# probabilists/azula

Measured on AMD Instinct MI355X. Metric: images/sec (whole node), DDIM-64 256x256 UNet, higher is better.
Workload: dtype f32 (f16x2 split: 2 half pieces per operand, 3 partial products, f32 accumulate)

## Files before the change

### azula_amd/_lib.py

```python

from __future__ import annotations

import ctypes as C
import functools
import os
import threading

import torch

_HERE = os.path.dirname(os.path.abspath(__file__))
LIB_PATH = os.environ.get("AZULA_AMD_LIB") or os.path.join(_HERE, "csrc", "libazula_amd.so")

c_f32p = C.c_void_p
c_stream = C.c_void_p


class AzStepCoef(C.Structure):
    _fields_ = [
        ("c_in", C.c_float),
        ("c_skip", C.c_float),
        ("c_out", C.c_float),
        ("c_time", C.c_float),
        ("alpha_t", C.c_float),
        ("alpha_s", C.c_float),
# ... 408 lines not shown
    "az_adm_precond_bwd_in_f32": [vp, vp, vp, vp, vp, vp, i32, i64, i64, f32, f32, c_stream],
    "az_linear_small_f32": [vp, i64, vp, i64, vp, vp, i64, i64, i64, i32, i32, c_stream],
    "az_gather_rows_f32": [vp, vp, vp, i64, i64, i64, c_stream],
    "az_gather_step_row_f32": [vp, vp, vp, i32, i64, i64, c_stream],
    "az_coef_c_time_f32": [vp, vp, c_stream],
    "az_groupnorm_stats_f32": [vp, vp, vp, i64, i64, i64, i64, i64, i32, i32, c_stream],
    "az_groupnorm_finalize_f32": [C.POINTER(AzNormFinalizeArgs), c_stream],
    "az_affine_act_f32": [vp, vp, vp, i64, vp, vp, i64, i64, i64, i64, i32, i32, c_stream],
    "az_rownorm_mod_f32": [vp, vp, vp, vp, vp, i64, i64, i64, i64, i64, i32, f32, c_stream],
    "az_rownorm_mod_h16": [vp, vp, vp, vp, vp, i64, i64, i64, i64, i64, i32, f32, i32, c_stream],
    "az_groupnorm_stats_h16": [vp, vp, vp, i64, i64, i64, i64, i64, i32, i32, i32, c_stream],
    "az_affine_act_h16": [vp, vp, vp, i64, vp, vp, i64, i64, i64, i64, i32, i32, i32, c_stream],
    "az_token_copy_f32": [vp, i64, i64, vp, i64, i64, i64, i64, i64, c_stream],
    "az_token_fill_f32": [vp, i64, i64, i64, vp, i64, vp, i64, i64, c_stream],
    "az_token_fill_h16": [vp, i64, i64, i64, vp, i64, vp, i64, i64, i32, c_stream],
    "az_timestep_embedding_f32": [vp, i64, vp, i64, i64, i32, f32, c_stream],
    "az_linear_small_grouped_f32": [vp, i32, i32, i64, i32, i32, c_stream],
    "az_conv2d_f32": [C.POINTER(AzConvArgs), c_stream],
    "az_conv2d_stem_f32": [C.POINTER(AzConvArgs), c_stream],
    "az_conv2d_bf16_f32": [C.POINTER(AzConvArgs), c_stream],
    "az_conv2d_x3_f32": [C.POINTER(AzConvArgs), c_stream],
    "az_conv2d_f16_f32": [C.POINTER(AzConvArgs), c_stream],
    "az_pack_conv_weight_half_f32": [vp, vp, i32, i32, i32, i32, i32, i32, i32, i32, c_stream],
    "az_pack_conv_weight_x3_f32": [vp, vp, i32, i32, i32, i32, i32, i32, i32, c_stream],
    "az_conv2d_suggest_splitk": [i64, i32, i32, i32],
    "az_conv2d_x3_suggest_splitk": [C.POINTER(AzConvArgs)],
    "az_conv2d_winograd_f32": [C.POINTER(AzConvArgs), c_stream],
    "az_conv2d_winograd_suggest_splitk": [i64, i32, i32, i32, i32],
    "az_winograd_pack_filter_f32": [vp, vp, i32, i32, i32, i32, i32, i32, c_stream],
    "az_conv2d_winograd_x3_f32": [C.POINTER(AzConvArgs), c_stream],
    "az_winograd_pack_filter_x3_f32": [vp, vp, i32, i32, i32, i32, i32, i32, c_stream],
    "az_winograd_x3_choose_block": [i32, i32, i32, i32, vp, vp, vp, vp],
    "az_winograd_x3_block_geometry": [i32, i32, i32, i32, i32, i32, i32, vp, vp],
    "az_conv2d_f16x2_f32": [C.POINTER(AzConvArgs), c_stream],
    "az_conv2d_winograd_f16x2_f32": [C.POINTER(AzConvArgs), c_stream],
    "az_pack_conv_weight_f16x2_f32": [vp, vp, i32, i32, i32, i32, i32, i32, i32, f32, c_stream],
    "az_winograd_pack_filter_f16x2_f32": [vp, vp, i32, i32, i32, i32, i32, i32, f32, c_stream],
    "az_f16x2_weight_scale": [f32, i32],
    "az_absmax_f32": [vp, vp, i64, c_stream],
    "az_absmax_from_moments_f32": [vp, vp, i64, c_stream],
    "az_conv2d_winograd4_f32": [C.POINTER(AzConvArgs), c_stream],
    "az_conv2d_winograd4_suggest_splitk": [i64, i32, i32, i32, i32],
    "az_winograd4_pack_filter_f32": [vp, vp, i32, i32, i32, i32, i32, i32, c_stream],
    "az_pack_conv_weight_f32": [vp, vp, i32, i32, i32, i32, i32, i32, i32, c_stream],
    "az_attention_f32": [C.POINTER(AzAttnArgs), c_stream],
    "az_attention_x3_f32": [C.POINTER(AzAttnArgs), c_stream],
    "az_attention_f16x2_f32": [C.POINTER(AzAttnArgs), c_stream],
    "az_attention_bf16_f32": [C.POINTER(AzAttnArgs), c_stream],
    "az_attention_f16_f32": [C.POINTER(AzAttnArgs), c_stream],
    "az_qk_prep_f32": [vp, vp, vp, vp, i64, i64, i32, i32, i64, i64, i64, i64, i64, i64, i32, i32, f32, vp, vp, c_stream],
    "az_qk_prep_w_f32": [vp, vp, vp, vp, i64, i64, i32, i32, i64, i64, i64, i64, i64, i64, i32, i32, f32, vp, vp, vp, vp, c_stream],
    "az_qk_prep_bwd_f32": [vp, vp, vp, vp, vp, vp, i64, i64, i32, i32, i64, i64, i64, i64, i64, i64, i64, i64, i64, i32, i32, f32, vp, vp,
                           c_stream],
    "az_qk_prep_bwd_w_f32": [vp, vp, vp, vp, vp, vp, i64, i64, i32, i32, i64, i64, i64, i64, i64, i64, i64, i64, i64, i32, i32, f32, vp,
                             vp, vp, vp, c_stream],
    "az_attention_bwd_f32": [C.POINTER(AzAttnBwdArgs), c_stream],
    "az_swiglu_f32": [vp, vp, i64, i64, i64, i64, c_stream],
    "az_patchify_f32": [vp, vp, vp, i64, i64, i64, i64, i64, i64, c_stream],
    "az_unpatchify_f32": [vp, vp, i64, i64, i64, i64, i64, i64, c_stream],
    "az_graph_begin": [c_stream],
    "az_graph_end": [c_stream, C.POINTER(vp)],
    "az_graph_launch": [vp, c_stream],
    "az_graph_destroy": [vp],
    "az_graph_num_nodes": [vp, C.POINTER(i64)],
    "az_transition_f64": [C.POINTER(AzTransitionArgs), c_stream],
    "az_step_row_f64": [vp, vp, vp, i32, i32, c_stream],
# ... 75 lines not shown
```

### azula_amd/csrc/conv.hip

```cpp
#include "conv_shared.h"
#include <cstdio>
#include <cstdlib>
#include <type_traits>

namespace {

constexpr int BM = 128;
constexpr int BN = 128;
constexpr int BK = 32;
constexpr int LDSS = 36;
constexpr int TILE_F = (BM + BN) * LDSS;

#include "igemm_kloop.inc"
struct ConvP {
  AzConvArgs a;
  int npix;
  int cin_s;
  int nkc0;
  int nkc1;
  int nk;
  int kps;
  int tiles_m;
  int tiles_n;
  int asm_loop;
// ... 2625 lines not shown

int az_winograd_x3_choose_block(int32_t batch, int32_t hin, int32_t win, int32_t whole, int32_t* rect_w, int32_t* rect_h,
                                int64_t* slots, int64_t* slots_run) {
  AZ_REQUIRE(rect_w && rect_h && slots && slots_run, AZ_E_NULL);
  AZ_REQUIRE(batch > 0 && hin > 0 && win > 0 && (int64_t)batch * hin * win < (1ll << 31), AZ_E_SHAPE);
  int rw, rh;
  int64_t run;
  *slots = x3_choose_block(batch, (hin + 1) / 2, (win + 1) / 2, whole != 0, rw, rh, run);
  *rect_w = rw, *rect_h = rh, *slots_run = run;
  return AZ_OK;
}

int az_winograd_x3_block_geometry(int32_t batch, int32_t hin, int32_t win, int32_t pad_mode, int32_t rect_w, int32_t rect_h,
                                  int32_t block, int32_t* slot_pix, int32_t* tile_info) {
  AZ_REQUIRE(slot_pix && tile_info, AZ_E_NULL);
  AZ_REQUIRE(batch > 0 && hin > 0 && win > 0 && (int64_t)batch * hin * win < (1ll << 31), AZ_E_SHAPE);
  AZ_REQUIRE(rect_h > 1 && x3_shape_ok(rect_w, rect_h), AZ_E_UNSUPPORTED);
  const int tiles_h = (hin + 1) / 2, tiles_w = (win + 1) / 2;
  AZ_REQUIRE(block >= 0 && block < (int64_t)batch * x3_rect_blocks_per_image(tiles_h, tiles_w, rect_w, rect_h), AZ_E_SHAPE);
  const X3RectGeom g = x3_rect_geom(block, tiles_h, tiles_w, rect_w, rect_h);
  for (int s = 0; s < 512; ++s) {
    int ih, iw;
    const bool ok = x3_rect_slot_pixel(g, s, hin, win, pad_mode, ih, iw);
    slot_pix[3 * s] = ok ? g.b : -1, slot_pix[3 * s + 1] = ok ? ih : -1, slot_pix[3 * s + 2] = ok ? iw : -1;
  }
  for (int j = 0; j < WT; ++j) {
    int th, tw, ps;
    const bool ok = x3_rect_tile(g, j, tiles_h, tiles_w, th, tw, ps);
    tile_info[4 * j] = ok ? g.b : -1, tile_info[4 * j + 1] = th, tile_info[4 * j + 2] = tw, tile_info[4 * j + 3] = ps;
  }
  return g.nslots;
}

static int winograd_x3_entry(const AzConvArgs* a, az_stream_t stream, bool h2) {
  WinoP p;
  int splitk = 1;
  const int prc = wino_prepare(a, 16, 16ll * WC * 16 * 3 * 2, p, splitk);
  if (prc != AZ_OK) return prc;
  AZ_REQUIRE(p.tiles_w >= 2, AZ_E_UNSUPPORTED);
  {
    const bool whole = p.a.gn_quads != nullptr;
    int rw, rh;
    int64_t run_slots;
    x3_choose_block(a->batch, p.tiles_h, p.tiles_w, whole, rw, rh, run_slots);
    if (const char* e = az_ab_env("AZ_X3_BLOCK")) {
      int ew = 0, eh = 0;
      if (sscanf(e, "%d,%d", &ew, &eh) == 2) {
        AZ_REQUIRE(x3_shape_ok(ew, eh) && !(whole && eh > 1 && (p.tiles_w % ew || p.tiles_h % eh)), AZ_E_UNSUPPORTED);
        rw = ew, rh = eh;
      }
    }
    if (rh > 1) {
      p.rect_w = rw, p.rect_h = rh;
      p.tblocks = a->batch * x3_rect_blocks_per_image(p.tiles_h, p.tiles_w, rw, rh);
      wino_order(p, 16);
    }
  }
  if (h2) AZ_REQUIRE(conv_pow2(a->w_scale), AZ_E_SHAPE);
  p.out_scale = h2 ? 1.f / a->w_scale : 1.f;
  if (h2) AZ_REQUIRE(AZ_ALIGNED16(a->in_absmax0) && AZ_ALIGNED16(a->in_absmax1) && (a->in_absmax0 || !a->in_absmax1), AZ_E_ALIGN);
  hipStream_t st = az_s(stream);
  int rc = azi_winograd_x3_launch(p, (unsigned)splitk, st, h2);
  if (rc != AZ_OK) return rc;
  if (splitk > 1) {
    ConvP cp;
    cp.a = p.a;
    cp.a.gn_quads = a->gn_quads;
    cp.npix = p.npix;
    rc = launch_splitk_reduce(cp, st);
  }
  return rc;
}

static void wino_order(WinoP& p, int wk) {
  int env_gt = 0, env_gc = 0;
  if (const char* e = az_ab_env("AZ_WINO_RECT")) sscanf(e, "%d,%d", &env_gt, &env_gc);
  int gt = env_gt > 0 ? env_gt : 8, gc = env_gt > 0 ? (env_gc > 0 ? env_gc : p.cblocks) : (wk == 16 ? 2 : 4);
  while (gc > 1 && p.cblocks % gc) gc >>= 1;
  if (env_gt <= 0) gt = 32 / gc;
  while (gt > 1 && p.tblocks % gt) gt >>= 1;
  if (p.cblocks % gc || p.tblocks % gt) gt = 1, gc = p.cblocks;
  p.gt = gt, p.gc = gc;
}

static int wino_prepare(const AzConvArgs* a, int wk, int64_t ustage_bytes, WinoP& p, int& splitk) {
  AZ_REQUIRE(a && a->src0 && a->weight && a->dst, AZ_E_NULL);
  AZ_REQUIRE(a->ksize == 3 && a->stride == 1 && a->pad == 1 && !a->aniso && a->src_dtype == 0 && a->dst_dtype == 0, AZ_E_UNSUPPORTED);
  AZ_REQUIRE(a->batch > 0 && a->hin > 0 && a->win > 0 && a->hout == a->hin && a->wout == a->win, AZ_E_SHAPE);
  AZ_REQUIRE(a->c0s > 0 && a->c0s % 4 == 0 && a->c1s % 4 == 0 && a->cout_s > 0 && a->cout_s % 4 == 0, AZ_E_SHAPE);
  AZ_REQUIRE((a->c1s == 0) == (a->src1 == nullptr), AZ_E_SHAPE);
// ... 31 lines not shown
  const int64_t npix64 = (int64_t)a->batch * a->hout * a->wout;
  AZ_REQUIRE(npix64 < (1ll << 31), AZ_E_SHAPE);
  if (a->gn_quads && a->splitk == 1) {
    const int64_t tiles_img = (int64_t)((a->hout + 1) / 2) * ((a->wout + 1) / 2);
    AZ_REQUIRE(!a->dst_nchw && a->cout_s % WC == 0 && tiles_img % WT == 0 && a->hout % 2 == 0 &&
                   a->wout % 2 == 0 && a->gn_chunks == tiles_img / WT,
               AZ_E_UNSUPPORTED);
  }

  p.a = *a;
  p.npix = (int)npix64;
  p.tiles_h = (a->hout + 1) / 2;
  p.tiles_w = (a->wout + 1) / 2;
  p.ntiles = a->batch * p.tiles_h * p.tiles_w;
  p.nkc0 = (a->c0s + wk - 1) / wk;
  p.nkc1 = (a->c1s + wk - 1) / wk;
  p.nk = p.nkc0 + p.nkc1;
  {
    const int64_t tiles_img = (int64_t)p.tiles_h * p.tiles_w;
    const int64_t span = (WT + tiles_img - 1) / tiles_img + 1;
    AZ_REQUIRE(span * a->h0 * a->w0 * a->c0s * 4 < (1ll << 31), AZ_E_SHAPE);
    AZ_REQUIRE(span * a->h1 * a->w1 * a->c1s * 4 < (1ll << 31), AZ_E_SHAPE);
  }
  splitk = a->splitk;
  if (splitk > p.nk) splitk = p.nk;
  p.kps = (p.nk + splitk - 1) / splitk;
  splitk = (p.nk + p.kps - 1) / p.kps;
  p.a.splitk = splitk;
  AZ_REQUIRE(!a->gn_quads || (a->splitk == 1) == (splitk == 1), AZ_E_UNSUPPORTED);
  if (splitk > 1) p.a.gn_quads = nullptr;
  p.cblocks = (a->cout_s + WC - 1) / WC;
  p.tblocks = (p.ntiles + WT - 1) / WT;
  p.rect_w = WT, p.rect_h = 1;
  wino_order(p, wk);
  AZ_REQUIRE((int64_t)p.nk * p.cblocks * ustage_bytes <= (1ll << 31), AZ_E_SHAPE);
  return AZ_OK;
}

int az_conv2d_winograd_suggest_splitk(int64_t batch, int32_t hout, int32_t wout, int32_t cout_s, int32_t cin_s) {
  const int64_t tiles = batch * ((hout + 1) / 2) * ((wout + 1) / 2);
  const int64_t blocks = ((tiles + WT - 1) / WT) * ((cout_s + WC - 1) / WC);
  const int64_t nk = (cin_s + WK - 1) / WK;
  int64_t want = (256 + blocks - 1) / blocks;
  int64_t maxs = nk / 8;
  if (maxs < 1) maxs = 1;
  if (want > maxs) want = maxs;
  if (want > 16) want = 16;
  if (blocks >= 192) want = 1;
  return (int)(want < 1 ? 1 : want);
}

int az_conv2d_winograd4_f32(const AzConvArgs* a, az_stream_t stream) {
  AZ_REQUIRE(a && a->src0 && a->weight && a->dst, AZ_E_NULL);
  AZ_REQUIRE(a->ksize == 3 && a->stride == 1 && a->pad == 1 && !a->aniso && a->src_dtype == 0 && a->dst_dtype == 0, AZ_E_UNSUPPORTED);
  AZ_REQUIRE(a->batch > 0 && a->hin > 0 && a->win > 0 && a->hout == a->hin && a->wout == a->win, AZ_E_SHAPE);
  AZ_REQUIRE(a->c0s > 0 && a->c0s % 4 == 0 && a->c1s % 4 == 0 && a->cout_s > 0 && a->cout_s % 4 == 0, AZ_E_SHAPE);
  AZ_REQUIRE((a->c1s == 0) == (a->src1 == nullptr), AZ_E_SHAPE);
  AZ_REQUIRE((a->act >= 0 && a->act <= 4) || a->act == 6, AZ_E_UNSUPPORTED);
  if (a->act == 6) AZ_REQUIRE(a->res && !a->gate && !a->dst_nchw && !a->gn_quads, AZ_E_UNSUPPORTED);
  if (a->act == 4) AZ_REQUIRE(!a->gate && !a->res && !a->dst_nchw && !a->gn_quads && a->cout_s % 8 == 0, AZ_E_UNSUPPORTED);
  AZ_REQUIRE(!a->in_affine && a->depth == 0, AZ_E_UNSUPPORTED);
  AZ_REQUIRE(!a->aniso || (a->up0_w >= 0 && a->up0_w <= 4 && a->up1_w >= 0 && a->up1_w <= 4), AZ_E_SHAPE);
  AZ_REQUIRE(a->up0 >= 0 && a->up0 <= 4 && ((a->hin + (1 << a->up0) - 1) >> a->up0) <= a->h0 &&
                 ((a->win + (1 << az_upw(a, a->up0, a->up0_w)) - 1) >> az_upw(a, a->up0, a->up0_w)) <= a->w0,
             AZ_E_SHAPE);
  if (a->src1)
// ... 73 lines not shown
```

### azula_amd/csrc/conv_shared.h

```cpp
#pragma once

#include "common.h"

namespace {

typedef float f32x16 __attribute__((ext_vector_type(16)));

__device__ __forceinline__ float4 ld4(const float* p) { return *reinterpret_cast<const float4*>(p); }


typedef unsigned int u32x4 __attribute__((ext_vector_type(4)));

__device__ __forceinline__ float4 buf_ld4(__amdgpu_buffer_rsrc_t rsrc, unsigned voff, unsigned soff) {
  const u32x4 v = __builtin_amdgcn_raw_buffer_load_b128(rsrc, (int)voff, (int)soff, 0);
  return __builtin_bit_cast(float4, v);
}

typedef float f32x2 __attribute__((ext_vector_type(2)));
typedef unsigned int u32x2 __attribute__((ext_vector_type(2)));

__device__ __forceinline__ f32x2 buf_ld2(__amdgpu_buffer_rsrc_t rsrc, unsigned voff, unsigned soff) {
  const u32x2 v = __builtin_amdgcn_raw_buffer_load_b64(rsrc, (int)voff, (int)soff, 0);
  return __builtin_bit_cast(f32x2, v);
}
// ... 323 lines not shown
  return az_fdiv(tiles_h + rh - 1, rh) * az_fdiv(tiles_w + rw - 1, rw);
}

__host__ __device__ __forceinline__ X3RectGeom x3_rect_geom(int tb, int tiles_h, int tiles_w, int rw, int rh) {
  X3RectGeom g;
  g.rw = rw, g.rh = rh;
  g.ws = 2 * rw + 2;
  g.nslots = (2 * rh + 2) * g.ws;
  const int bw = az_fdiv(tiles_w + rw - 1, rw);
  const int bpi = az_fdiv(tiles_h + rh - 1, rh) * bw;
  g.b = az_fdiv(tb, bpi);
  g.rb = tb - g.b * bpi;
  const int by = az_fdiv(g.rb, bw);
  g.th0 = by * rh;
  g.tw0 = (g.rb - by * bw) * rw;
  return g;
}

__host__ __device__ __forceinline__ bool x3_rect_slot_pixel(const X3RectGeom& g, int s, int hin, int win, int pad_mode, int& ih, int& iw) {
  const int r = az_fdiv(s, g.ws);
  ih = wrap_coord(2 * g.th0 - 1 + r, hin, pad_mode);
  iw = wrap_coord(2 * g.tw0 - 1 + (s - r * g.ws), win, pad_mode);
  return s < g.nslots && (unsigned)ih < (unsigned)hin && (unsigned)iw < (unsigned)win;
}

__host__ __device__ __forceinline__ bool x3_rect_tile(const X3RectGeom& g, int j, int tiles_h, int tiles_w, int& th, int& tw, int& pslot) {
  const int jy = az_fdiv(j, g.rw), jx = j - jy * g.rw;
  th = g.th0 + jy;
  tw = g.tw0 + jx;
  pslot = 2 * jy * g.ws + 2 * jx;
  return th < tiles_h && tw < tiles_w;
}


}

struct WinoP {
  AzConvArgs a;
  int npix;
  int tiles_h, tiles_w, ntiles;
  int nkc0, nkc1, nk;
  int kps;
  int cblocks;
  int tblocks;
  int gt, gc;
  int rect_w, rect_h;
  float out_scale;
};
```

### azula_amd/csrc/wino_x3.hip

```cpp
#include "conv_shared.h"

#include <cstdlib>
#include <type_traits>

namespace {

typedef __bf16 bf16x8 __attribute__((ext_vector_type(8)));
typedef _Float16 f16x8 __attribute__((ext_vector_type(8)));

constexpr int XT = 64;
constexpr int XC = 64;
constexpr int XK = 16;
constexpr int X_ROW = XK * 4;
constexpr int X_FREQ = XT * X_ROW;
constexpr int X_HALF = 8 * X_FREQ;
constexpr int X_STAGE = 2 * X_HALF;
constexpr int X_SLOTS = 768;
constexpr int X_SLOT = 64;
constexpr int X_DOFF1 = X_STAGE + X_SLOTS * X_SLOT;
constexpr int X_OT = 2 * XC + 4;
constexpr int X_EPI_BYTES = (4 * XT * X_OT + 3 * XT + 384) * 4;
constexpr int X_LDS_BYTES = X_DOFF1 + 512 * 32 > X_EPI_BYTES ? X_DOFF1 + 512 * 32 : X_EPI_BYTES;
static_assert(X_LDS_BYTES >= X_DOFF1 + 512 * 32 && X_LDS_BYTES >= 4 * 128 * 64 * 4, "the epilogue reuses the K loop's LDS");
constexpr int XU_STEP_BYTES = 16 * XC * XK * 3 * 2;
static_assert(4 * X_SLOTS <= 6 * 512, "six staging pieces per thread");
static_assert(X_LDS_BYTES <= 160 * 1024, "one workgroup per CU");

template <int AFF, bool TAIL, bool H2 = false, bool RECT = false>
__global__ __launch_bounds__(512, 2) void conv_winograd_x3_kernel(WinoP p) {
  extern __shared__ __attribute__((aligned(16))) float wsm[];
  char* const smem = reinterpret_cast<char*>(wsm);
  const AzConvArgs& a = p.a;
  const int tid = threadIdx.x;
  const int lane = tid & 63;
  const int wave = tid >> 6;
  const int wxi = wave & 3;
  const int wk = wave >> 2;
  const int l31 = lane & 31;
  const int h = lane >> 5;

  const int nwg = gridDim.x;
  const int bid = blockIdx.x;
  const int xq = nwg >> 3, xr = nwg & 7, xcd = bid & 7;
  const int wg = (xcd < xr ? xcd * (xq + 1) : xr * (xq + 1) + (xcd - xr) * xq) + (bid >> 3);
  const int rsz = p.gt * p.gc;
  const int rect = wg / rsz, rin = wg - rect * rsz;
  const int rcols = p.cblocks / p.gc;
  const int rrow = rect / rcols;
  const int rin_c = rin / p.gt;
  const int tb = rrow * p.gt + (rin - rin_c * p.gt);
  const int cb = (rect - rrow * rcols) * p.gc + rin_c;
  const int t0 = tb * XT;
  const int tiles_img = p.tiles_h * p.tiles_w;
  X3RectGeom rg = {};
  if constexpr (RECT) rg = x3_rect_geom(tb, p.tiles_h, p.tiles_w, p.rect_w, p.rect_h);
  const int b_first = RECT ? rg.b : t0 / tiles_img;

  const int kt_begin = blockIdx.y * p.kps;
  const int kt_end = min(p.nk, kt_begin + p.kps);
  const float pin = H2 ? az_f16x2_in_scale(a.in_absmax0, a.in_absmax1, 4.f, lane) : 1.f;
  const float pin2k = pin * 2048.f;
// ... 136 lines not shown
#pragma unroll
      for (int c = 0; c < 4; ++c) rv[4 * r + c] = *reinterpret_cast<const f32x2*>(patch + r * prow + c * X_SLOT);
  };
  const __amdgpu_buffer_rsrc_t raf = __builtin_amdgcn_make_buffer_rsrc(
      (void*)(AFF != 0 ? a.in_affine : nullptr), 0, AFF != 0 ? (unsigned)(2 * a.batch * a.c0s * 4) : 0u, 0x00020000);
  const unsigned af_voff = (unsigned)(((b_first + (v_b < 0 ? 0 : v_b)) * a.c0s + vq * 2) * 4);
  const unsigned af_shift = (unsigned)(a.batch * a.c0s * 4);
  f32x2 af_sc = {0.f, 0.f}, af_sh = {0.f, 0.f};
  auto affine_load = [&](int kt) __attribute__((always_inline)) {
    if constexpr (AFF != 0) {
      const bool kv = !TAIL || kt * XK + vq * 2 < a.c0s;
      af_sc = buf_ld2(raf, kv ? af_voff : OOB, (unsigned)(kt * XK * 4));
      af_sh = buf_ld2(raf, kv ? af_voff : OOB, (unsigned)(kt * XK * 4) + af_shift);
    }
  };
  auto affine = [&]() __attribute__((always_inline)) {
    if constexpr (AFF != 0) {
#pragma unroll
      for (int i = 0; i < 16; ++i) {
        f32x2 v = rv[i] * af_sc + af_sh;
        if constexpr (AFF == 2) v = f32x2{az_silu(v.x), az_silu(v.y)};
        rv[i] = (vmask >> i) & 1u ? v : f32x2{0.f, 0.f};
      }
    }
  };
  auto row_transform = [&](int c) __attribute__((always_inline)) {
    const f32x2 d0 = rv[c], d1 = rv[4 + c], d2 = rv[8 + c], d3 = rv[12 + c];
    rv[c] = d0 - d2;
    rv[4 + c] = d1 + d2;
    rv[8 + c] = d2 - d1;
    rv[12 + c] = d1 - d3;
  };
  const int vrow = vj * X_ROW + (((vq >> 1) ^ ((vj >> 2) & 3)) * 16) + (vq & 1) * 8;
  auto nu_store = [&](int hs, int xi) __attribute__((always_inline)) {
    const f32x2 u0 = rv[4 * xi], u1 = rv[4 * xi + 1], u2 = rv[4 * xi + 2], u3 = rv[4 * xi + 3];
    char* dst = smem + hs * X_HALF + vrow + (2 * xi) * X_FREQ;
    *reinterpret_cast<f32x2*>(dst) = hs == 0 ? u0 - u2 : u2 - u1;
    *reinterpret_cast<f32x2*>(dst + X_FREQ) = hs == 0 ? u1 + u2 : u1 - u3;
  };
  const unsigned u_lane = (unsigned)(lane * 16);
  constexpr bool H2_DERIVE = true;
  uint4 ua[2][3];
  typedef _Float16 f16x8v __attribute__((ext_vector_type(8)));
  auto derive_u2 = [&]() __attribute__((always_inline)) {
#pragma unroll
    for (int ch = 0; ch < 2; ++ch) ua[ch][2] = __builtin_bit_cast(uint4, __builtin_bit_cast(f16x8v, ua[ch][0]) * (_Float16)0.00048828125f);
  };
  auto load_u = [&](int kt, int f, int pl) __attribute__((always_inline)) {
    const unsigned soff =
        (unsigned)__builtin_amdgcn_readfirstlane((int)((((int64_t)kt * p.cblocks + cb) * 8 + wave) * (12 * 1024) + f * (6 * 1024)));
#pragma unroll
    for (int ch = 0; ch < 2; ++ch) ua[ch][pl] = __builtin_bit_cast(uint4, buf_ld4(rw, u_lane + (unsigned)((ch * 3 + pl) * 1024), soff));
  };

  f32x16 acc[8];
#pragma unroll
  for (int f = 0; f < 8; ++f)
#pragma unroll
    for (int r = 0; r < 16; ++r) acc[f][r] = 0.f;

  const int fragB = (2 * wxi + wk) * X_FREQ + l31 * X_ROW;
  const int fsw = (l31 >> 2) & 3;
  float xf[2][8];
  unsigned fw[2][3][4];
  auto frag_read = [&](int hs, int th) __attribute__((always_inline)) {
    const char* vb = smem + hs * X_HALF + fragB + th * (32 * X_ROW);
    const float4 lo = *reinterpret_cast<const float4*>(vb + (((2 * h) ^ fsw) * 16));
    const float4 hi = *reinterpret_cast<const float4*>(vb + (((2 * h + 1) ^ fsw) * 16));
    xf[th][0] = lo.x, xf[th][1] = lo.y, xf[th][2] = lo.z, xf[th][3] = lo.w;
// ... 11 lines not shown
      xf[th][i] = x - __builtin_bit_cast(float, __builtin_bit_cast(unsigned, x) & 0xFFFF0000u);
    }
  };
  constexpr int PA[6] = {H2 ? 1 : 2, H2 ? 0 : 1, H2 ? 2 : 0, 1, 0, 0};
  constexpr int PB[6] = {0, 0, H2 ? 1 : 0, 1, 1, 2};
  auto mf = [&](int f, int k) __attribute__((always_inline)) {
    const int t = k >> 2, th = (k >> 1) & 1, ch = k & 1;
    f32x16& c = acc[4 * f + 2 * ch + th];
    uint4 bw = make_uint4(fw[th][PB[t]][0], fw[th][PB[t]][1], fw[th][PB[t]][2], fw[th][PB[t]][3]);
    if constexpr (H2) c = __builtin_amdgcn_mfma_f32_32x32x16_f16(__builtin_bit_cast(f16x8, ua[ch][PA[t]]), __builtin_bit_cast(f16x8, bw), c, 0, 0, 0);
    else c = __builtin_amdgcn_mfma_f32_32x32x16_bf16(__builtin_bit_cast(bf16x8, ua[ch][PA[t]]), __builtin_bit_cast(bf16x8, bw), c, 0, 0, 0);
  };
  typedef _Float16 h2v __attribute__((ext_vector_type(2)));
  auto h_piece = [&](int th) __attribute__((always_inline)) {
#pragma unroll
    for (int j = 0; j < 4; ++j) {
      const f32x2 x = {xf[th][2 * j], xf[th][2 * j + 1]};
      const f32x2 v = x * pin;
      fw[th][0][j] = __builtin_bit_cast(unsigned, __builtin_convertvector(v, h2v));
      const f32x2 t = x * pin2k;
      xf[th][2 * j] = t.x, xf[th][2 * j + 1] = t.y;
    }
  };
  auto l_piece = [&](int th) __attribute__((always_inline)) {
#pragma unroll
    for (int j = 0; j < 4; ++j) {
      const h2v hh = __builtin_bit_cast(h2v, fw[th][0][j]);
      const h2v l = {(_Float16)__builtin_fmaf((float)hh.x, -2048.f, xf[th][2 * j]), (_Float16)__builtin_fmaf((float)hh.y, -2048.f, xf[th][2 * j + 1])};
      fw[th][1][j] = __builtin_bit_cast(unsigned, l);
    }
  };

#define XS_FENCE __builtin_amdgcn_sched_barrier(0)
  auto phase = [&](auto HS, int kt, int ktn) __attribute__((always_inline)) {
    constexpr int hs = decltype(HS)::value;
    constexpr int ob = 1 - hs;
    const int ktu = hs == 0 ? kt : ktn;
    if constexpr (H2) {
      h_piece(0); XS_FENCE;
      if constexpr (hs == 0) {
        mf(hs, 0); h_piece(1); XS_FENCE;
        mf(hs, 1); nu_store(ob, 0); nu_store(ob, 1); XS_FENCE;
        mf(hs, 2); nu_store(ob, 2); nu_store(ob, 3); gl(ktn, 0); gl(ktn, 1); gl(ktn, 2); XS_FENCE;
        mf(hs, 3); gl(ktn, 3); gl(ktn, 4); gl(ktn, 5); load_u(ktu, ob, 1); XS_FENCE;
        mf(hs, 4); l_piece(0); XS_FENCE;
        mf(hs, 5); l_piece(1); if constexpr (H2_DERIVE) derive_u2(); XS_FENCE;
        mf(hs, 6); XS_FENCE;
        mf(hs, 7); load_u(ktu, ob, 0); XS_FENCE;
        mf(hs, 8); gs(0); XS_FENCE;
        mf(hs, 9); gs(1); gs(2); XS_FENCE;
        mf(hs, 10); gs(3); gs(4); XS_FENCE;
        mf(hs, 11); gs(5);
      } else {
        mf(hs, 0); h_piece(1); affine_load(ktn); XS_FENCE;
        mf(hs, 1); patch_rows(ktn, 0, 2); XS_FENCE;
        mf(hs, 2); patch_rows(ktn, 2, 4); XS_FENCE;
        mf(hs, 3); l_piece(0); load_u(ktu, ob, 1); XS_FENCE;
        mf(hs, 4); l_piece(1); if constexpr (H2_DERIVE) derive_u2(); XS_FENCE;
        affine();
        mf(hs, 5); row_transform(0); row_transform(1); XS_FENCE;
        mf(hs, 6); row_transform(2); row_transform(3); XS_FENCE;
        mf(hs, 7); load_u(ktu, ob, 0); XS_FENCE;
        mf(hs, 8); nu_store(ob, 0); XS_FENCE;
        mf(hs, 9); nu_store(ob, 1); XS_FENCE;
        mf(hs, 10); nu_store(ob, 2); XS_FENCE;
        mf(hs, 11); nu_store(ob, 3);
      }
      if constexpr (!H2_DERIVE) load_u(ktu, ob, 2);
// ... 27 lines not shown
    } else {
      mf(hs, 0); piece(1, 0); XS_FENCE;
      mf(hs, 1); affine_load(ktn); remainder(0, 0, 2); XS_FENCE;
      mf(hs, 2); remainder(0, 2, 4); XS_FENCE;
      mf(hs, 3); remainder(1, 0, 2); XS_FENCE;
      mf(hs, 4); remainder(1, 2, 4); load_u(ktu, ob, 2); XS_FENCE;
      mf(hs, 5); piece(0, 1); XS_FENCE;
      mf(hs, 6); piece(1, 1); XS_FENCE;
      mf(hs, 7); remainder(0, 0, 2); XS_FENCE;
      mf(hs, 8); remainder(0, 2, 4); XS_FENCE;
      mf(hs, 9); remainder(1, 0, 2); XS_FENCE;
      mf(hs, 10); remainder(1, 2, 4); XS_FENCE;
      mf(hs, 11); piece(0, 2); piece(1, 2); XS_FENCE;
      mf(hs, 12); patch_rows(ktn, 0, 2); XS_FENCE;
      mf(hs, 13); patch_rows(ktn, 2, 4); XS_FENCE;
      mf(hs, 14); XS_FENCE;
      mf(hs, 15); XS_FENCE;
      mf(hs, 16); load_u(ktu, ob, 1); XS_FENCE;
      affine();
      mf(hs, 17); row_transform(0); row_transform(1); XS_FENCE;
      mf(hs, 18); row_transform(2); row_transform(3); XS_FENCE;
      mf(hs, 19); nu_store(ob, 0); XS_FENCE;
      mf(hs, 20); nu_store(ob, 1); XS_FENCE;
      mf(hs, 21); nu_store(ob, 2); XS_FENCE;
      mf(hs, 22); nu_store(ob, 3); XS_FENCE;
      mf(hs, 23);
    }
    load_u(ktu, ob, 0);
    }
    __syncthreads();
    frag_read(ob, 0); frag_read(ob, 1);
    XS_FENCE;
  };

  if (kt_begin < kt_end) {
#pragma unroll
    for (int m = 0; m < 6; ++m) gl(kt_begin, m);
    if constexpr (H2) {
      XS_FENCE; load_u(kt_begin, 0, 1); XS_FENCE; load_u(kt_begin, 0, 0); XS_FENCE;
      if constexpr (!H2_DERIVE) { load_u(kt_begin, 0, 2); XS_FENCE; }
    } else {
      XS_FENCE; load_u(kt_begin, 0, 2); XS_FENCE; load_u(kt_begin, 0, 1); XS_FENCE; load_u(kt_begin, 0, 0); XS_FENCE;
    }
#pragma unroll
    for (int m = 0; m < 6; ++m) gs(m);
    __syncthreads();
    affine_load(kt_begin);
    patch_rows(kt_begin, 0, 4);
    affine();
#pragma unroll
    for (int c = 0; c < 4; ++c) row_transform(c);
#pragma unroll
    for (int xi = 0; xi < 4; ++xi) nu_store(0, xi);
    __syncthreads();
    frag_read(0, 0); frag_read(0, 1);
    if (wave >= 4) __builtin_amdgcn_s_setprio(1);
#pragma unroll 1
    for (int kt = kt_begin; kt < kt_end; ++kt) {
      const int ktn = min(kt + 1, kt_end - 1);
      if (ktn >= p.nkc0 && cur_src == 0) switch_source();
      phase(std::integral_constant<int, 0>{}, kt, ktn);
      phase(std::integral_constant<int, 1>{}, kt, ktn);
    }
    __builtin_amdgcn_s_setprio(0);
  }
  __syncthreads();
#undef XS_FENCE
  if constexpr (H2) {
    const float osc = __fdiv_rn(p.out_scale, pin);
#pragma unroll
    for (int q = 0; q < 8; ++q) acc[q] = acc[q] * osc;
  }

  if (wk == 0) {
    asm volatile("" ::: "memory");
#pragma unroll
    for (int q = 0; q < 4; ++q) {
      acc[q] = acc[q] + acc[4 + q];
      acc[4 + q] = -acc[4 + q];
    }
  } else {
    asm volatile("" ::: "memory");
#pragma unroll
    for (int q = 0; q < 4; ++q) acc[4 + q] = acc[q] - acc[4 + q];
  }
  {
    float4* hand = reinterpret_cast<float4*>(wsm) + wxi * (32 * 64) + lane;
    if (wk == 1) {
#pragma unroll
      for (int q = 0; q < 8; ++q)
#pragma unroll
        for (int g = 0; g < 4; ++g) hand[(q * 4 + g) * 64] = make_float4(acc[q][4 * g], acc[q][4 * g + 1], acc[q][4 * g + 2], acc[q][4 * g + 3]);
    }
    __syncthreads();
    if (wk == 0) {
// ... 84 lines not shown
    a2 = (a2 + b2) + d * d * half_n;
  };
  chan(am, a2, __shfl_xor(am, 16), __shfl_xor(a2, 16), 16.f);
  chan(am, a2, __shfl_xor(am, 32), __shfl_xor(a2, 32), 32.f);
  float* sh = reinterpret_cast<float*>(tinfo + 3 * XT);
  if (lane < 16) {
    sh[wave * 16 + lane] = am;
    sh[128 + wave * 16 + lane] = a2;
  }
  __syncthreads();
  if (tid < 16) {
    float wm[8], w2[8];
#pragma unroll
    for (int k = 0; k < 8; ++k) {
      wm[k] = sh[k * 16 + tid];
      w2[k] = sh[128 + k * 16 + tid];
    }
    float hn = 64.f;
#pragma unroll
    for (int o = 1; o < 8; o <<= 1, hn *= 2.f)
#pragma unroll
      for (int k = 0; k < 8; k += 2 * o) chan(wm[k], w2[k], wm[k + o], w2[k + o], hn);
    const int chunk = RECT ? rg.rb : (t0 - b_first * tiles_img) / XT;
    float* out = a.gn_quads + ((((int64_t)b_first * a.gn_chunks + chunk) * (a.cout_s / 4)) + (cb * (XC / 4) + tid)) * 4;
    out[0] = 1024.f;
    out[1] = wm[0];
    out[2] = w2[0];
    out[3] = 0.f;
  }
}

}

template <int AFF, bool TAIL, bool H2, bool RECT>
static int launch_x3(const WinoP& p, unsigned splitk, hipStream_t st) {
  static std::atomic<uint64_t> lds_set{0};
  hipError_t e = az_max_dynamic_lds((const void*)conv_winograd_x3_kernel<AFF, TAIL, H2, RECT>, X_LDS_BYTES, lds_set);
  if (e != hipSuccess) return (int)e;
  hipLaunchKernelGGL((conv_winograd_x3_kernel<AFF, TAIL, H2, RECT>), dim3((unsigned)((int64_t)p.cblocks * p.tblocks), splitk), dim3(512), X_LDS_BYTES,
                     st, p);
  return az_launch_status();
}

template <bool H2, bool RECT>
static int launch_x3_mode(const WinoP& p, unsigned splitk, hipStream_t st) {
  const bool tail = (p.a.c0s % XK) != 0 || (p.a.c1s % XK) != 0;
  const int aff = !p.a.in_affine ? 0 : (p.a.in_act == 0 ? 1 : 2);
  switch (aff * 2 + (tail ? 1 : 0)) {
    case 0: return launch_x3<0, false, H2, RECT>(p, splitk, st);
    case 1: return launch_x3<0, true, H2, RECT>(p, splitk, st);
    case 2: return launch_x3<1, false, H2, RECT>(p, splitk, st);
    case 3: return launch_x3<1, true, H2, RECT>(p, splitk, st);
    case 4: return launch_x3<2, false, H2, RECT>(p, splitk, st);
    default: return launch_x3<2, true, H2, RECT>(p, splitk, st);
  }
}

__attribute__((visibility("hidden"))) int azi_winograd_x3_launch(const WinoP& p, unsigned splitk, hipStream_t st, bool h2) {
  if (p.rect_h > 1) {
    if (p.rect_w * p.rect_h != XT || (2 * p.rect_w + 2) * (2 * p.rect_h + 2) > 512) return AZ_E_SHAPE;
    return h2 ? launch_x3_mode<true, true>(p, splitk, st) : launch_x3_mode<false, true>(p, splitk, st);
  }
  return h2 ? launch_x3_mode<true, false>(p, splitk, st) : launch_x3_mode<false, false>(p, splitk, st);
}
```

### include/azula_amd.h

```cpp
#ifndef AZULA_AMD_H
#define AZULA_AMD_H

#include <stdint.h>

#ifdef __cplusplus
extern "C" {
#endif

#define AZ_VERSION 1

enum {
  AZ_OK = 0,
  AZ_E_NULL = -1,
  AZ_E_SHAPE = -2,
  AZ_E_ALIGN = -3,
  AZ_E_UNSUPPORTED = -4
};

typedef void* az_stream_t;

int az_version(void);
const char* az_error_string(int code);

typedef struct AzStepCoef {
// ... 316 lines not shown
  int32_t src_dtype;
  int32_t depth;
  int32_t depth_shift;
  int32_t qk_head_dim;
  int32_t qk_heads;
  int32_t qk_tokens;
  int32_t qk_rmsnorm;
  float qk_eps;
  int32_t qk_reserved;
  const float* qk_q_weight;
  const float* qk_k_weight;
  const float* qk_rope_cos;
  const float* qk_rope_sin;
  int32_t depth_wrap;
  int32_t dst_dtype;
  float w_scale;
  int32_t reserved1;
  const float* in_absmax0;
  const float* in_absmax1;
} AzConvArgs;
int az_conv2d_f32(const AzConvArgs* args, az_stream_t stream);
int az_conv2d_stem_f32(const AzConvArgs* args, az_stream_t stream);
int az_conv2d_bf16_f32(const AzConvArgs* args, az_stream_t stream);
int az_conv2d_f16_f32(const AzConvArgs* args, az_stream_t stream);
int az_conv2d_x3_f32(const AzConvArgs* args, az_stream_t stream);
int az_conv2d_x3_suggest_splitk(const AzConvArgs* args);
int az_conv2d_winograd_f32(const AzConvArgs* args, az_stream_t stream);
int az_conv2d_winograd_suggest_splitk(int64_t batch, int32_t hout, int32_t wout, int32_t cout_s, int32_t cin_s);
int az_conv2d_winograd_x3_f32(const AzConvArgs* args, az_stream_t stream);
int az_winograd_x3_choose_block(int32_t batch, int32_t hin, int32_t win, int32_t whole, int32_t* rect_w, int32_t* rect_h,
                                int64_t* slots, int64_t* slots_run);
int az_winograd_x3_block_geometry(int32_t batch, int32_t hin, int32_t win, int32_t pad_mode, int32_t rect_w, int32_t rect_h,
                                  int32_t block, int32_t* slot_pix, int32_t* tile_info);
#define AZ_F16X2_IN_SCALE 0.0625f
int az_conv2d_f16x2_f32(const AzConvArgs* args, az_stream_t stream);
int az_conv2d_winograd_f16x2_f32(const AzConvArgs* args, az_stream_t stream);
float az_f16x2_weight_scale(float amax, int32_t winograd);
#define AZ_ABSMAX_SLOTS 256
int az_absmax_f32(float* slots, const float* x, int64_t n, az_stream_t stream);
int az_absmax_from_moments_f32(float* slots, const float* partials, int64_t count, az_stream_t stream);
int az_conv2d_winograd4_f32(const AzConvArgs* args, az_stream_t stream);
int az_conv2d_winograd4_suggest_splitk(int64_t batch, int32_t hout, int32_t wout, int32_t cout_s, int32_t cin_s);
int az_conv2d_suggest_splitk(int64_t npix, int32_t cout_s, int32_t cin_s, int32_t ksize);
int az_pack_conv_weight_f32(float* dst, const float* src, int32_t cout, int32_t cin, int32_t ks, int32_t cout_s,
                            int32_t cin0, int32_t c0s, int32_t cin_s, az_stream_t stream);

typedef struct AzAttnArgs {
  const float* q;
  const float* k;
  const float* v;
  float* out;
  int32_t batch, heads, tokens, head_dim;
  int64_t q_bstride, q_tstride, q_hstride;
  int64_t k_bstride, k_tstride, k_hstride;
  int64_t v_bstride, v_tstride, v_hstride;
  int64_t o_bstride, o_tstride, o_hstride;
  float scale;
  int32_t qk_rmsnorm;
  float eps;
  int32_t norm_dim;
  const float* rope_cos;
  const float* rope_sin;
  const float* q_weight;
  const float* k_weight;
  const uint8_t* mask;
  int64_t mask_bstride, mask_hstride;
// ... 118 lines not shown
```

Before: 4.697.

## Skip structurally zero Winograd input-transform work for upsampled x3 conv sources

Adds a UPS specialization of the Winograd x3 kernel used when the input source(s) are nearest-upsampled. For these, parts of the input transform are structurally redundant. Once the K loop reaches the upsampled source, it splits into per-wave variants that skip some consume or next-load phases and write fewer transformed values to LDS. A host query and an env switch (AZ_X3_UPS) are added. This cuts redundant transform and MMA work in decoder convs, at the cost of more kernel instantiations and a riskier per-wave divergent schedule.

Result: faster. 4.755 (median of 6 runs) (+1.2%).

```diff
diff --git a/azula_amd/_lib.py b/azula_amd/_lib.py
--- a/azula_amd/_lib.py
+++ b/azula_amd/_lib.py
@@ -464,6 +464,7 @@
     "az_winograd_pack_filter_x3_f32": [vp, vp, i32, i32, i32, i32, i32, i32, c_stream],
     "az_winograd_x3_choose_block": [i32, i32, i32, i32, vp, vp, vp, vp],
     "az_winograd_x3_block_geometry": [i32, i32, i32, i32, i32, i32, i32, vp, vp],
+    "az_winograd_x3_structured_mask": [C.POINTER(AzConvArgs), vp, vp],
     "az_conv2d_f16x2_f32": [C.POINTER(AzConvArgs), c_stream],
     "az_conv2d_winograd_f16x2_f32": [C.POINTER(AzConvArgs), c_stream],
     "az_pack_conv_weight_f16x2_f32": [vp, vp, i32, i32, i32, i32, i32, i32, i32, f32, c_stream],
diff --git a/azula_amd/csrc/conv.hip b/azula_amd/csrc/conv.hip
--- a/azula_amd/csrc/conv.hip
+++ b/azula_amd/csrc/conv.hip
@@ -2681,6 +2681,19 @@
   return g.nslots;
 }
 
+static int x3_launch_mask(const AzConvArgs& a) {
+  if (const char* e = az_ab_env("AZ_X3_UPS"))
+    if (e[0] == '0') return 0;
+  return x3_structured_mask(a);
+}
+
+int az_winograd_x3_structured_mask(const AzConvArgs* a, int32_t* mask, int32_t* launch_mask) {
+  AZ_REQUIRE(a && mask && launch_mask, AZ_E_NULL);
+  *mask = x3_structured_mask(*a);
+  *launch_mask = x3_launch_mask(*a);
+  return AZ_OK;
+}
+
 static int winograd_x3_entry(const AzConvArgs* a, az_stream_t stream, bool h2) {
   WinoP p;
   int splitk = 1;
@@ -2705,6 +2718,7 @@
       wino_order(p, 16);
     }
   }
+  p.ups = x3_launch_mask(p.a);
   if (h2) AZ_REQUIRE(conv_pow2(a->w_scale), AZ_E_SHAPE);
   p.out_scale = h2 ? 1.f / a->w_scale : 1.f;
   if (h2) AZ_REQUIRE(AZ_ALIGNED16(a->in_absmax0) && AZ_ALIGNED16(a->in_absmax1) && (a->in_absmax0 || !a->in_absmax1), AZ_E_ALIGN);
@@ -2802,6 +2816,7 @@
   p.cblocks = (a->cout_s + WC - 1) / WC;
   p.tblocks = (p.ntiles + WT - 1) / WT;
   p.rect_w = WT, p.rect_h = 1;
+  p.ups = 0;
   wino_order(p, wk);
   AZ_REQUIRE((int64_t)p.nk * p.cblocks * ustage_bytes <= (1ll << 31), AZ_E_SHAPE);
   return AZ_OK;
diff --git a/azula_amd/csrc/conv_shared.h b/azula_amd/csrc/conv_shared.h
--- a/azula_amd/csrc/conv_shared.h
+++ b/azula_amd/csrc/conv_shared.h
@@ -379,6 +379,13 @@
   return th < tiles_h && tw < tiles_w;
 }
 
+__host__ __device__ __forceinline__ int x3_structured_mask(const AzConvArgs& a) {
+  if (a.aniso || a.in_affine || ((a.hin | a.win) & 1) || (a.pad_mode != 0 && a.pad_mode != 1)) return 0;
+  const int m0 = a.up0 >= 1 ? 1 : 0;
+  const int m1 = a.src1 && a.up1 >= 1 ? 2 : 0;
+  if (a.src1 && !m1) return 0;
+  return m0 | m1;
+}
 
 }
 
@@ -393,4 +400,5 @@
   int gt, gc;
   int rect_w, rect_h;
   float out_scale;
+  int ups;
 };
diff --git a/azula_amd/csrc/wino_x3.hip b/azula_amd/csrc/wino_x3.hip
--- a/azula_amd/csrc/wino_x3.hip
+++ b/azula_amd/csrc/wino_x3.hip
@@ -26,7 +26,7 @@
 static_assert(4 * X_SLOTS <= 6 * 512, "six staging pieces per thread");
 static_assert(X_LDS_BYTES <= 160 * 1024, "one workgroup per CU");
 
-template <int AFF, bool TAIL, bool H2 = false, bool RECT = false>
+template <int AFF, bool TAIL, bool H2 = false, bool RECT = false, bool UPS = false>
 __global__ __launch_bounds__(512, 2) void conv_winograd_x3_kernel(WinoP p) {
   extern __shared__ __attribute__((aligned(16))) float wsm[];
   char* const smem = reinterpret_cast<char*>(wsm);
@@ -229,9 +229,14 @@
     rv[12 + c] = d1 - d3;
   };
   const int vrow = vj * X_ROW + (((vq >> 1) ^ ((vj >> 2) & 3)) * 16) + (vq & 1) * 8;
-  auto nu_store = [&](int hs, int xi) __attribute__((always_inline)) {
+  auto nu_store = [&](int hs, int xi, bool pst = false) __attribute__((always_inline)) {
+    if (pst && xi == 2) return;
     const f32x2 u0 = rv[4 * xi], u1 = rv[4 * xi + 1], u2 = rv[4 * xi + 2], u3 = rv[4 * xi + 3];
     char* dst = smem + hs * X_HALF + vrow + (2 * xi) * X_FREQ;
+    if (pst && hs == 1) {
+      *reinterpret_cast<f32x2*>(dst + X_FREQ) = u1 - u3;
+      return;
+    }
     *reinterpret_cast<f32x2*>(dst) = hs == 0 ? u0 - u2 : u2 - u1;
     *reinterpret_cast<f32x2*>(dst + X_FREQ) = hs == 0 ? u1 + u2 : u1 - u3;
   };
@@ -309,8 +314,27 @@
   };
 
 #define XS_FENCE __builtin_amdgcn_sched_barrier(0)
-  auto phase = [&](auto HS, int kt, int ktn) __attribute__((always_inline)) {
+    auto body = [&](auto HS, auto CONS_, auto NEXT_, auto PST_, int kt, int ktn) __attribute__((always_inline)) {
     constexpr int hs = decltype(HS)::value;
+    constexpr bool CONS = decltype(CONS_)::value, NEXT = decltype(NEXT_)::value, PST = decltype(PST_)::value;
+    const auto& mf_ = mf;
+    const auto& h_piece_ = h_piece;
+    const auto& l_piece_ = l_piece;
+    const auto& derive_u2_ = derive_u2;
+    const auto& piece_ = piece;
+    const auto& remainder_ = remainder;
+    const auto& load_u_ = load_u;
+    const auto& frag_read_ = frag_read;
+    const auto& nu_store_ = nu_store;
+    auto mf = [&](int f, int k) __attribute__((always_inline)) { if constexpr (CONS) mf_(f, k); };
+    auto h_piece = [&](int th) __attribute__((always_inline)) { if constexpr (CONS) h_piece_(th); };
+    auto l_piece = [&](int th) __attribute__((always_inline)) { if constexpr (CONS) l_piece_(th); };
+    auto derive_u2 = [&]() __attribute__((always_inline)) { if constexpr (CONS) derive_u2_(); };
+    auto piece = [&](int th, int pl) __attribute__((always_inline)) { if constexpr (CONS) piece_(th, pl); };
+    auto remainder = [&](int th, int j0, int j1) __attribute__((always_inline)) { if constexpr (CONS) remainder_(th, j0, j1); };
+    auto load_u = [&](int ku, int f, int pl) __attribute__((always_inline)) { if constexpr (NEXT) load_u_(ku, f, pl); };
+    auto frag_read = [&](int half, int th) __attribute__((always_inline)) { if constexpr (NEXT) frag_read_(half, th); };
+    auto nu_store = [&](int half, int xi) __attribute__((always_inline)) { nu_store_(half, xi, PST); };
     constexpr int ob = 1 - hs;
     const int ktu = hs == 0 ? kt : ktn;
     if constexpr (H2) {
@@ -404,7 +428,15 @@
     frag_read(ob, 0); frag_read(ob, 1);
     XS_FENCE;
   };
-
+  auto steps = [&](auto C0, auto N0, auto C1, auto N1, auto PST_, int k0, int k1) __attribute__((always_inline)) {
+#pragma unroll 1
+    for (int kt = k0; kt < k1; ++kt) {
+      const int ktn = min(kt + 1, kt_end - 1);
+      if (ktn >= p.nkc0 && cur_src == 0) switch_source();
+      body(std::integral_constant<int, 0>{}, C0, N0, PST_, kt, ktn);
+      body(std::integral_constant<int, 1>{}, C1, N1, PST_, kt, ktn);
+    }
+  };
   if (kt_begin < kt_end) {
 #pragma unroll
     for (int m = 0; m < 6; ++m) gl(kt_begin, m);
@@ -427,12 +459,18 @@
     __syncthreads();
     frag_read(0, 0); frag_read(0, 1);
     if (wave >= 4) __builtin_amdgcn_s_setprio(1);
-#pragma unroll 1
-    for (int kt = kt_begin; kt < kt_end; ++kt) {
-      const int ktn = min(kt + 1, kt_end - 1);
-      if (ktn >= p.nkc0 && cur_src == 0) switch_source();
-      phase(std::integral_constant<int, 0>{}, kt, ktn);
-      phase(std::integral_constant<int, 1>{}, kt, ktn);
+    constexpr std::true_type T{};
+    constexpr std::false_type F{};
+    if constexpr (!UPS) {
+      steps(T, T, T, T, F, kt_begin, kt_end);
+    } else {
+      const int ks = (p.ups & 1) ? kt_begin : max(kt_begin, min(kt_end, p.nkc0));
+      const int swave = __builtin_amdgcn_readfirstlane(wave);
+      const bool xi2 = (swave & 3) == 2, k0 = !xi2 && swave < 4;
+      steps(T, T, T, T, F, kt_begin, ks);
+      steps(T, T, T, T, T, ks, xi2 || k0 ? ks : kt_end);
+      steps(T, F, F, T, T, ks, k0 ? kt_end : ks);
+      steps(F, F, F, F, T, ks, xi2 ? kt_end : ks);
     }
     __builtin_amdgcn_s_setprio(0);
   }
@@ -583,12 +621,12 @@
 
 }
 
-template <int AFF, bool TAIL, bool H2, bool RECT>
+template <int AFF, bool TAIL, bool H2, bool RECT, bool UPS = false>
 static int launch_x3(const WinoP& p, unsigned splitk, hipStream_t st) {
   static std::atomic<uint64_t> lds_set{0};
-  hipError_t e = az_max_dynamic_lds((const void*)conv_winograd_x3_kernel<AFF, TAIL, H2, RECT>, X_LDS_BYTES, lds_set);
+  hipError_t e = az_max_dynamic_lds((const void*)conv_winograd_x3_kernel<AFF, TAIL, H2, RECT, UPS>, X_LDS_BYTES, lds_set);
   if (e != hipSuccess) return (int)e;
-  hipLaunchKernelGGL((conv_winograd_x3_kernel<AFF, TAIL, H2, RECT>), dim3((unsigned)((int64_t)p.cblocks * p.tblocks), splitk), dim3(512), X_LDS_BYTES,
+  hipLaunchKernelGGL((conv_winograd_x3_kernel<AFF, TAIL, H2, RECT, UPS>), dim3((unsigned)((int64_t)p.cblocks * p.tblocks), splitk), dim3(512), X_LDS_BYTES,
                      st, p);
   return az_launch_status();
 }
@@ -597,6 +635,10 @@
 static int launch_x3_mode(const WinoP& p, unsigned splitk, hipStream_t st) {
   const bool tail = (p.a.c0s % XK) != 0 || (p.a.c1s % XK) != 0;
   const int aff = !p.a.in_affine ? 0 : (p.a.in_act == 0 ? 1 : 2);
+  if (p.ups) {
+    if (aff != 0 || p.ups != x3_structured_mask(p.a)) return AZ_E_SHAPE;
+    return tail ? launch_x3<0, true, H2, RECT, true>(p, splitk, st) : launch_x3<0, false, H2, RECT, true>(p, splitk, st);
+  }
   switch (aff * 2 + (tail ? 1 : 0)) {
     case 0: return launch_x3<0, false, H2, RECT>(p, splitk, st);
     case 1: return launch_x3<0, true, H2, RECT>(p, splitk, st);
diff --git a/include/azula_amd.h b/include/azula_amd.h
--- a/include/azula_amd.h
+++ b/include/azula_amd.h
@@ -372,6 +372,7 @@
                                 int64_t* slots, int64_t* slots_run);
 int az_winograd_x3_block_geometry(int32_t batch, int32_t hin, int32_t win, int32_t pad_mode, int32_t rect_w, int32_t rect_h,
                                   int32_t block, int32_t* slot_pix, int32_t* tile_info);
+int az_winograd_x3_structured_mask(const AzConvArgs* args, int32_t* mask, int32_t* launch_mask);
 #define AZ_F16X2_IN_SCALE 0.0625f
 int az_conv2d_f16x2_f32(const AzConvArgs* args, az_stream_t stream);
 int az_conv2d_winograd_f16x2_f32(const AzConvArgs* args, az_stream_t stream);
```
